# kawshik8/GAN-Image-Captioning

Hardware: AMD Instinct MI355X
Metric: captions/sec (G+D train step) (higher is better)
Workload: dtype bf16; 1 GPU; cfg2: adversarial G+D step, batch 64/GPU, 224x224 images, caption len 20, V=10000, E=H=512, 1-layer LSTM G, CNN-seq D (R=64,F=900), ResNet-50-shaped encoder, --conditional-gan 1; global_batch=64, caption_len=20, image_size=224, vocab=10000, conditional_gan=1, encoder=resnet50, step_impl=fused, parallelism=dp1

## Files before the change

### gan-image-captioning_amd/_lib.py

```python
from __future__ import annotations

import ctypes as C
import os

import torch

from . import build as _build

MAX_LAYERS = 4
MAX_CONVS = 8
F32, BF16 = 0, 1
LOSS_TYPES = {"standard": 0, "JS": 1, "KL": 2, "hinge": 3, "tv": 4, "rsgan": 5}

c_float_p = C.POINTER(C.c_float)
c_void_p = C.c_void_p


class DecoderDims(C.Structure):
    _fields_ = [(n, C.c_int32) for n in ("B", "L", "V", "E", "H", "NL", "dtype")]


class DecoderParams(C.Structure):
    _fields_ = [("embed", c_void_p), ("w_ih", c_void_p * MAX_LAYERS), ("w_hh", c_void_p * MAX_LAYERS),
                ("b_ih", c_void_p * MAX_LAYERS), ("b_hh", c_void_p * MAX_LAYERS), ("w_out", c_void_p), ("b_out", c_void_p)]
# ... 88 lines not shown
                ("o2l_w", c_void_p), ("o2l_b", c_void_p)]


class DiscGrads(C.Structure):
    _fields_ = DiscParams._fields_


class DiscShadow(C.Structure):
    _fields_ = [("emb", c_void_p), ("hw_w", c_void_p), ("f2o_w", c_void_p), ("hw_w_t", c_void_p)]


class DiscState(C.Structure):
    _fields_ = [("emb", c_void_p), ("pooled", c_void_p), ("argmax", c_void_p), ("hpre", c_void_p),
                ("keep", c_void_p), ("ydrop", c_void_p), ("feat", c_void_p)]


class DiscBwdWs(C.Structure):
    _fields_ = [("dfeat", c_void_p), ("dh", c_void_p), ("dydrop", c_void_p), ("dpooled", c_void_p), ("demb", c_void_p)]


class BnRunningDesc(C.Structure):
    _fields_ = [("stats", c_void_p), ("running_mean", c_void_p), ("running_var", c_void_p), ("count", C.c_float),
                ("momentum", C.c_float), ("C", C.c_int32), ("nrep", C.c_int32)]


_P = C.POINTER
_SIGNATURES = {
    "gic_abi_version": (C.c_int, []),
    "gic_last_error": (C.c_char_p, []),
    "gic_debug_route_only": (None, [C.c_int]),
    "gic_debug_last_route": (C.c_char_p, []),
    "gic_gemm": (C.c_int, [c_void_p, c_void_p, c_void_p, C.c_int, C.c_int, C.c_int, C.c_int64, C.c_int64, C.c_int64,
                           C.c_int, C.c_int, C.c_int, C.c_int, c_void_p, C.c_int, C.c_float, c_void_p]),
    "gic_cast2d": (C.c_int, [c_void_p, C.c_int, C.c_int64, c_void_p, C.c_int, C.c_int64, C.c_int64, C.c_int64, c_void_p]),
    "gic_decoder_state_bytes": (C.c_int, [_P(DecoderDims), c_void_p]),
    "gic_decoder_bwd_ws_bytes": (C.c_int, [_P(DecoderDims), c_void_p]),
    "gic_disc_state_bytes": (C.c_int, [_P(DiscDims), c_void_p]),
    "gic_disc_bwd_ws_bytes": (C.c_int, [_P(DiscDims), c_void_p]),
    "gic_decoder_prepare": (C.c_int, [_P(DecoderDims), _P(DecoderParams), _P(DecoderShadow), c_void_p]),
    "gic_decoder_sample_fwd": (C.c_int, [_P(DecoderDims), _P(DecoderParams), _P(DecoderShadow), _P(DecoderState), c_void_p,
                                         c_void_p, C.c_uint64, C.c_float, C.c_int, c_void_p, c_void_p, _P(DecoderSampleOpts), c_void_p]),
    "gic_decoder_forward_tf": (C.c_int, [_P(DecoderDims), _P(DecoderParams), _P(DecoderShadow), _P(DecoderState), c_void_p, c_void_p,
                                         c_void_p, C.c_int, c_void_p, C.c_uint64, C.c_float, C.c_int, c_void_p, c_void_p, c_void_p,
                                         c_void_p, c_void_p, c_void_p]),
    "gic_decoder_forward_tf_bwd": (C.c_int, [_P(DecoderDims), _P(DecoderParams), _P(DecoderShadow), _P(DecoderState), _P(DecoderBwdWs),
                                             c_void_p, c_void_p, c_void_p, C.c_int, c_void_p, C.c_float, C.c_int, _P(DecoderGrads), c_void_p]),
    "gic_decoder_sample_bwd": (C.c_int, [_P(DecoderDims), _P(DecoderParams), _P(DecoderShadow), _P(DecoderState),
                                         _P(DecoderBwdWs), c_void_p, c_void_p, c_void_p, C.c_float, C.c_int,
                                         _P(DecoderGrads), C.c_int, c_void_p, c_void_p]),
    "gic_step_scalars_set": (C.c_int, [c_void_p, _P(StepScalars), c_void_p]),
    "gic_debug_decoder_step": (None, [C.c_int]),
    "gic_decoder_fused_rollout_rows": (C.c_int, [_P(DecoderDims), c_void_p]),
    "gic_decoder_beam_ws_bytes": (C.c_int, [_P(DecoderDims), C.c_int32, c_void_p]),
    "gic_decoder_beam_search": (C.c_int, [_P(DecoderDims), _P(DecoderParams), _P(DecoderShadow), _P(DecoderBeamOpts), c_void_p, c_void_p,
                                          c_void_p, c_void_p, c_void_p, c_void_p]),
    "gic_attn_prepare": (C.c_int, [_P(AttnDims), _P(AttnParams), _P(AttnShadow), c_void_p]),
    "gic_attn_sample_fwd": (C.c_int, [_P(AttnDims), _P(AttnParams), _P(AttnShadow), _P(AttnState), c_void_p, c_void_p, c_void_p, C.c_uint64,
                                      C.c_float, C.c_int, c_void_p, c_void_p, c_void_p, c_void_p, c_void_p, C.c_int, c_void_p]),
    "gic_attn_sample_bwd": (C.c_int, [_P(AttnDims), _P(AttnParams), _P(AttnShadow), _P(AttnState), _P(AttnBwdWs), c_void_p, c_void_p, c_void_p,
                                      c_void_p, C.c_float, C.c_int, _P(AttnGrads), c_void_p, c_void_p]),
    "gic_attn_beam_ws_bytes": (C.c_int, [_P(AttnDims), C.c_int32, c_void_p]),
    "gic_attn_beam_search": (C.c_int, [_P(AttnDims), _P(AttnParams), _P(AttnShadow), _P(DecoderBeamOpts), c_void_p, c_void_p, c_void_p,
                                       c_void_p, c_void_p, c_void_p, c_void_p, c_void_p]),
    "gic_decoder_diverse_beam_search": (C.c_int, [_P(DecoderDims), _P(DecoderParams), _P(DecoderShadow), _P(DiverseBeamOpts), c_void_p,
                                                  c_void_p, c_void_p, c_void_p, c_void_p, c_void_p]),
    "gic_attn_diverse_beam_search": (C.c_int, [_P(AttnDims), _P(AttnParams), _P(AttnShadow), _P(DiverseBeamOpts), c_void_p, c_void_p,
# ... 125 lines not shown
```

### gan-image-captioning_amd/csrc/decoder.hip

```cpp
#include <stdlib.h>

#include "../../include/gicap.h"
#include "decoder_step.h"
#include "kernels.h"

namespace gic {
namespace {

__device__ __forceinline__ float sigmoidf_(float x) { return 1.f / (1.f + expf(-x)); }

template <typename TA>
__global__ void lstm_pointwise_fwd_kernel(const float* __restrict__ gpre, const float* __restrict__ c_prev,
                                          float* __restrict__ gates, float* __restrict__ c_new,
                                          TA* __restrict__ h_next, long ld_next,
                                          TA* __restrict__ h_up, long ld_up,
                                          TA* __restrict__ h_out, long ld_out,
                                          int B, int H) {
  const int idx = blockIdx.x * blockDim.x + threadIdx.x;
  if (idx >= B * H) return;
  const int b = idx / H, j = idx % H;
  const float* g = gpre + (long)b * 4 * H;
  const float i_ = sigmoidf_(g[j]);
  const float f_ = sigmoidf_(g[H + j]);
  const float g_ = tanhf(g[2 * H + j]);
  const float o_ = sigmoidf_(g[3 * H + j]);
  const float c = f_ * c_prev[idx] + i_ * g_;
  const float h = o_ * tanhf(c);
  if (gates) {
    float* go = gates + (long)b * 4 * H;
    go[j] = i_; go[H + j] = f_; go[2 * H + j] = g_; go[3 * H + j] = o_;
  }
  c_new[idx] = c;
  h_next[(long)b * ld_next + j] = from_f32<TA>(h);
  if (h_up) h_up[(long)b * ld_up + j] = from_f32<TA>(h);
  if (h_out) h_out[(long)b * ld_out + j] = from_f32<TA>(h);
}

// ... 536 lines not shown
  } else {
  for (int l = 0; l < NL; ++l) {
    GIC_PROPAGATE(fill_zero(ws->dxh[l], (size_t)(L + 1) * B * c.ldx(l) * sizeof(float), stream));
  }
  for (int t = L - 1; t >= 0; --t) {
    for (int l = NL - 1; l >= 0; --l) {
      const long ld = c.ldx(l);
      const float* dh_a;
      long ld_a;
      if (l == NL - 1) { dh_a = ws->dhout + (long)t * H; ld_a = (long)L * H; }
      else { dh_a = ws->dxh[l + 1] + (long)t * B * c.ldx(l + 1); ld_a = c.ldx(l + 1); }
      const float* dh_b = ws->dxh[l] + (long)(t + 1) * B * ld + c.din(l);
      TA* dg = (TA*)ws->dgates[l] + (long)t * B * 4 * H;
      hipLaunchKernelGGL((lstm_pointwise_bwd_kernel<TA>), dim3(pw_grid), dim3(256), 0, stream, dh_a, ld_a, dh_b, ld,
                         (const float*)(st->gates[l] + (long)t * B * 4 * H), (const float*)(st->c[l] + (long)t * B * H),
                         (const float*)(st->c[l] + (long)(t + 1) * B * H), ws->dc[l], dg, B, H);
      GIC_CHECK_LAUNCH("lstm_pointwise_bwd");
      GemmDesc g;
      g.A = dg; g.lda = 4 * H; g.a_kc = 1;
      if (S->wcat_t[l]) { g.B = S->wcat_t[l]; g.ldb = 4 * H; g.b_kc = 1; }
      else { g.B = S->wcat[l]; g.ldb = ld; g.b_kc = 0; }
      g.C = ws->dxh[l] + (long)t * B * ld; g.ldc = ld; g.c_zeroed = 1;
      g.M = B; g.N = (int)ld; g.K = 4 * H; g.in_dtype = c.dt; g.out_dtype = DT_F32;
      GIC_PROPAGATE(gemm(g, stream));
    }
  }
  }
  for (int l = 0; l < NL; ++l) {
    const long ld = c.ldx(l);
    GemmDesc w;
    w.A = ws->dgates[l]; w.lda = 4 * H; w.a_kc = 0; w.b_kc = 0; w.ldb = ld;
    w.M = 4 * H; w.K = (int)BL; w.in_dtype = c.dt; w.out_dtype = DT_F32;
    w.B = st->xh[l]; w.N = c.din(l); w.C = G->w_ih[l]; w.ldc = c.din(l);
    GIC_PROPAGATE(gemm(w, stream));
    w.B = (const TA*)st->xh[l] + c.din(l); w.N = H; w.C = G->w_hh[l]; w.ldc = H;
    GIC_PROPAGATE(gemm(w, stream));
    GIC_PROPAGATE(colsum(ws->dgates[l], c.dt, 4 * H, BL, 4 * H, G->b_ih[l], G->b_hh[l], 0, stream));
  }
  GIC_PROPAGATE(cast2d(ws->dxh[0], DT_F32, c.ldx(0), G->features, DT_F32, E, B, E, stream));
  return GIC_OK;
}

__global__ void embed_scatter_time_kernel(const float* __restrict__ dxh0, long ld, const int64_t* __restrict__ ids, long ids_stride,
                                          float* __restrict__ dw, int B, int L, int E, int V) {
  const long total = (long)(L - 1) * B * E;
  for (long i = (long)blockIdx.x * blockDim.x + threadIdx.x; i < total; i += (long)gridDim.x * blockDim.x) {
    const int e = (int)(i % E);
    const long r = i / E;
    const int b = (int)(r % B);
    const int t = (int)(r / B) + 1;
    long id = ids[(long)b * ids_stride + (t - 1)];
    id = id < 0 ? 0 : (id >= V ? V - 1 : id);
    atomicAdd(&dw[id * E + e], dxh0[((long)t * B + b) * ld + e]);
  }
}

}

int decoder_output_bwd(int dt, int B, int L, int V, int H, const void* probs, const void* d_out, float temperature, const float* t_dev, int pretrain,
                       void* dlogits_ws, const void* wout, const void* hout, float* dhout, float* d_wout, float* d_bout, hipStream_t stream) {
  const long BL = (long)B * L;
  const void* dlog = pretrain ? d_out : (const void*)dlogits_ws;
  if (!pretrain) {
    const bool al = ((((uintptr_t)probs) | ((uintptr_t)d_out) | ((uintptr_t)dlogits_ws)) & 15) == 0;
    if (dt == DT_F32) {
      if (al && V % 4 == 0 && V <= 256 * 8 * 4)
        hipLaunchKernelGGL((softmax_bwd_vec_kernel<float, 8>), dim3((unsigned)BL), dim3(256), 0, stream, (const float*)probs, (const float*)d_out,
                           (float*)dlogits_ws, temperature, t_dev, V);
      else
        hipLaunchKernelGGL((softmax_bwd_kernel<float>), dim3((unsigned)BL), dim3(256), 0, stream, (const float*)probs, (const float*)d_out,
                           (float*)dlogits_ws, temperature, t_dev, V);
    } else {
      if (al && V % 8 == 0 && V <= 256 * 5 * 8)
        hipLaunchKernelGGL((softmax_bwd_vec_kernel<bf16_t, 5>), dim3((unsigned)BL), dim3(256), 0, stream, (const bf16_t*)probs, (const bf16_t*)d_out,
                           (bf16_t*)dlogits_ws, temperature, t_dev, V);
      else if (al && V % 8 == 0 && V <= 256 * 8 * 8)
        hipLaunchKernelGGL((softmax_bwd_vec_kernel<bf16_t, 8>), dim3((unsigned)BL), dim3(256), 0, stream, (const bf16_t*)probs, (const bf16_t*)d_out,
                           (bf16_t*)dlogits_ws, temperature, t_dev, V);
      else
        hipLaunchKernelGGL((softmax_bwd_kernel<bf16_t>), dim3((unsigned)BL), dim3(256), 0, stream, (const bf16_t*)probs, (const bf16_t*)d_out,
                           (bf16_t*)dlogits_ws, temperature, t_dev, V);
    }
    GIC_CHECK_LAUNCH("softmax_bwd");
  }
  GemmDesc g;
  g.A = dlog; g.lda = V; g.a_kc = 1; g.B = wout; g.ldb = H; g.b_kc = 0; g.C = dhout; g.ldc = H;
  g.M = (int)BL; g.N = H; g.K = V; g.in_dtype = dt; g.out_dtype = DT_F32;
  GIC_PROPAGATE(gemm(g, stream));
  GemmDesc w;
  w.A = dlog; w.lda = V; w.a_kc = 0; w.B = hout; w.ldb = H; w.b_kc = 0; w.C = d_wout; w.ldc = H;
  w.M = V; w.N = H; w.K = (int)BL; w.in_dtype = dt; w.out_dtype = DT_F32;
  GIC_PROPAGATE(gemm(w, stream));
  return colsum(dlog, dt, V, BL, V, d_bout, nullptr, 0, stream);
}

int lstm_pointwise_fwd(int dt, const float* gpre, const float* c_prev, float* c_new, void* h_next, long ld_next, void* h_up, long ld_up,
                       int rows, int H, hipStream_t stream) {
  const dim3 grid((unsigned)cdiv((long)rows * H, 256));
  if (dt == DT_F32)
    hipLaunchKernelGGL((lstm_pointwise_fwd_kernel<float>), grid, dim3(256), 0, stream, gpre, c_prev, (float*)nullptr, c_new, (float*)h_next, ld_next,
                       (float*)h_up, ld_up, (float*)nullptr, 0l, rows, H);
  else
    hipLaunchKernelGGL((lstm_pointwise_fwd_kernel<bf16_t>), grid, dim3(256), 0, stream, gpre, c_prev, (float*)nullptr, c_new, (bf16_t*)h_next,
                       ld_next, (bf16_t*)h_up, ld_up, (bf16_t*)nullptr, 0l, rows, H);
  GIC_CHECK_LAUNCH("lstm_pointwise_fwd");
  return GIC_OK;
}

int embed_scatter_time(const float* dx, long ld, const int64_t* ids, float* d_embed, int B, int L, int E, int V, hipStream_t stream, long ids_stride) {
  if (ids_stride <= 0) ids_stride = L;
  GIC_PROPAGATE(fill_zero(d_embed, (size_t)V * E * sizeof(float), stream));
  if (L > 1 && det_mode())
    return det_scatter(dx, DT_F32, ld, B, ids, B, ids_stride, 1, (long)(L - 1) * B, d_embed, E, 1, E, V, stream);
  if (L > 1) {
    const long total = (long)(L - 1) * B * E;
    const int grid = (int)((total + 255) / 256 > 2048 ? 2048 : (total + 255) / 256);
    hipLaunchKernelGGL(embed_scatter_time_kernel, dim3(grid), dim3(256), 0, stream, dx, ld, ids, ids_stride, d_embed, B, L, E, V);
    GIC_CHECK_LAUNCH("embed_scatter_time");
  }
  return GIC_OK;
}

}

using namespace gic;
// ... 316 lines not shown
```

### gan-image-captioning_amd/csrc/disc.hip

```cpp
#include <stdlib.h>
#include "../../include/gicap.h"
#include "kernels.h"

namespace gic {
namespace {

constexpr int kMaxTaps = 32;
constexpr int kOutDim = 100;
constexpr int kOutPad = 104;

struct ConvMeta {
  int nconv, F, Fp, s;
  int fsize[GIC_MAX_CONVS], nfilt[GIC_MAX_CONVS], foff[GIC_MAX_CONVS];
  const float* w[GIC_MAX_CONVS];
  const float* b[GIC_MAX_CONVS];
  float* dw[GIC_MAX_CONVS];
  float* db[GIC_MAX_CONVS];
};

__device__ __forceinline__ int conv_of(const ConvMeta& cm, int col) {
  int k = 0;
  while (k + 1 < cm.nconv && col >= cm.foff[k + 1]) ++k;
  return k;
}

__global__ void disc_emb_gather_kernel(const float* __restrict__ w, const int64_t* __restrict__ ids, float* __restrict__ emb,
                                       long rows, int De, int V) {
  const long total = rows * De;
  for (long i = (long)blockIdx.x * blockDim.x + threadIdx.x; i < total; i += (long)gridDim.x * blockDim.x) {
    const long r = i / De;
    const int e = (int)(i % De);
    long id = ids[r];
    id = id < 0 ? 0 : (id >= V ? V - 1 : id);
    emb[i] = w[(long)e * V + id];
  }
// ... 698 lines not shown
               const float* d_logits, const gic_disc_grads* G, int accumulate, void* d_inp, long ld_dinp, hipStream_t stream) {
  const long MR = c.rowsBR;
  if (G && !accumulate) {
    GIC_PROPAGATE(fill_zero(G->o2l_w, kOutDim * sizeof(float), stream));
    GIC_PROPAGATE(fill_zero(G->o2l_b, sizeof(float), stream));
    for (int k = 0; k < c.cm.nconv; ++k) {
      GIC_PROPAGATE(fill_zero(G->conv_w[k], (size_t)c.cm.nfilt[k] * c.cm.fsize[k] * c.s * sizeof(float), stream));
      GIC_PROPAGATE(fill_zero(G->conv_b[k], (size_t)c.cm.nfilt[k] * sizeof(float), stream));
    }
    if (inp_ids) GIC_PROPAGATE(fill_zero(G->emb, (size_t)c.De * c.V * sizeof(float), stream));
  }
  const bool det = G && det_mode();
  const long dy_floats = MR * c.Fp;
  int out_blocks = 256;
  if (det && (long)out_blocks * (kOutDim + 1) > dy_floats) out_blocks = (int)(dy_floats / (kOutDim + 1));
  if (out_blocks < 1) out_blocks = 1;
  const bool out_part = det && out_blocks > 1;
  hipLaunchKernelGGL((disc_out_bwd_kernel<TA>), dim3(out_blocks), dim3(256), 0, stream, d_logits, (const float*)st->feat, P->o2l_w,
                     (TA*)ws->dfeat, G ? G->o2l_w : nullptr, G ? G->o2l_b : nullptr, MR, out_part ? ws->dydrop : nullptr);
  GIC_CHECK_LAUNCH("disc_out_bwd");
  if (out_part) {
    hipLaunchKernelGGL(disc_out_fold_kernel, dim3(1), dim3(128), 0, stream, (const float*)ws->dydrop, out_blocks, G->o2l_w, G->o2l_b);
    GIC_CHECK_LAUNCH("disc_out_fold");
  }
  {
    GemmDesc g;
    g.A = ws->dfeat; g.lda = kOutPad; g.a_kc = 1; g.B = S->f2o_w; g.ldb = c.Fp; g.b_kc = 0; g.C = ws->dydrop; g.ldc = c.Fp;
    g.M = (int)MR; g.N = c.Fp; g.K = kOutPad; g.in_dtype = c.dt; g.out_dtype = DT_F32;
    GIC_PROPAGATE(gemm(g, stream));
    if (G) {
      GemmDesc w;
      w.A = ws->dfeat; w.lda = kOutPad; w.a_kc = 0; w.B = st->ydrop; w.ldb = c.Fp; w.b_kc = 0; w.C = G->f2o_w; w.ldc = c.F;
      w.M = kOutDim; w.N = c.F; w.K = (int)MR; w.in_dtype = c.dt; w.out_dtype = DT_F32; w.accumulate = accumulate;
      GIC_PROPAGATE(gemm(w, stream));
      GIC_PROPAGATE(colsum(ws->dfeat, c.dt, kOutPad, MR, kOutDim, G->f2o_b, nullptr, accumulate, stream, (float*)ws->dh,
                           (long)(MR * c.Fp * dtype_size(c.dt) / sizeof(float))));
    }
  }
  const bool hb_vec = MR * c.Fp / 8 < (1l << 31) && ((((uintptr_t)ws->dydrop) | ((uintptr_t)st->hpre) | ((uintptr_t)st->pooled) | ((uintptr_t)ws->dh) |
                                                     ((uintptr_t)ws->dpooled)) & 15) == 0 && (!train || (((uintptr_t)st->keep) & 7) == 0);
  if (hb_vec)
    hipLaunchKernelGGL((disc_highway_bwd_vec_kernel<TA>), dim3(grid1d(MR * c.Fp / 8)), dim3(256), 0, stream, (const float*)ws->dydrop,
                       train ? (const uint8_t*)st->keep : nullptr, c.keep_scale(train), (const float*)st->hpre,
                       (const TA*)st->pooled, (TA*)ws->dh, ws->dpooled, (unsigned)(MR * c.Fp / 8), c.F, c.Fp / 8);
  else
    hipLaunchKernelGGL((disc_highway_bwd_kernel<TA>), dim3(grid1d(MR * c.Fp)), dim3(256), 0, stream, (const float*)ws->dydrop,
                       train ? (const uint8_t*)st->keep : nullptr, c.keep_scale(train), (const float*)st->hpre,
                       (const TA*)st->pooled, (TA*)ws->dh, ws->dpooled, MR, c.F, c.Fp);
  GIC_CHECK_LAUNCH("disc_highway_bwd");
  {
    GemmDesc g;
    g.A = ws->dh; g.lda = c.Fp; g.a_kc = 1; g.B = S->hw_w_t ? S->hw_w_t : S->hw_w; g.ldb = c.Fp; g.b_kc = S->hw_w_t ? 1 : 0;
    g.C = ws->dpooled; g.ldc = c.Fp;
    g.M = (int)MR; g.N = c.Fp; g.K = c.Fp; g.in_dtype = c.dt; g.out_dtype = DT_F32; g.accumulate = 1;
    GIC_PROPAGATE(gemm(g, stream));
    if (G) {
      GemmDesc w;
      w.A = ws->dh; w.lda = c.Fp; w.a_kc = 0; w.B = st->pooled; w.ldb = c.Fp; w.b_kc = 0; w.C = G->hw_w; w.ldc = c.F;
      w.M = c.F; w.N = c.F; w.K = (int)MR; w.in_dtype = c.dt; w.out_dtype = DT_F32; w.accumulate = accumulate;
      GIC_PROPAGATE(gemm(w, stream));
      GIC_PROPAGATE(colsum(ws->dh, c.dt, c.Fp, MR, c.F, G->hw_b, nullptr, accumulate, stream, ws->dydrop, (long)(MR * c.Fp)));
    }
  }
  if (G) {
    int gy = cdiv(MR, 4 * 8);
    gy = gy > 64 ? 64 : gy;
    int mt = 0;
    for (int k = 0; k < c.cm.nconv; ++k) mt = c.cm.fsize[k] * c.s > mt ? c.cm.fsize[k] * c.s : mt;
    static const bool no_lds = getenv("GIC_NO_DISC_BWDW_LDS") != nullptr;
    const bool lds = mt <= 8 && c.s == 1 && c.R <= 64 && c.R <= c.De && MR % c.R == 0 && c.L <= 64 && !no_lds;
    const int ncap = (int)(MR / c.R);
    const int mt1 = (mt <= 8 ? 8 : kMaxTaps) + 1;
    int rows_y = lds ? (ncap < 64 ? ncap : 64) : gy;
    if (det && (long)rows_y * c.F * mt1 > dy_floats) rows_y = (int)(dy_floats / ((long)c.F * mt1));
    if (rows_y < 1) rows_y = 1;
    gy = lds ? gy : rows_y;
    float* part = det && rows_y > 1 ? ws->dydrop : nullptr;
    if (lds) {
      hipLaunchKernelGGL((disc_conv_pool_bwd_w_lds_kernel<TA, 8>), dim3(cdiv(c.F, 64), rows_y), dim3(256),
                         (size_t)c.R * ((c.L + 8) | 1) * sizeof(float), stream, (const float*)ws->dpooled, (const TA*)st->pooled,
                         (const uint8_t*)st->argmax, (const float*)st->emb, c.cm, c.L, c.De, c.R, ncap, part);
    } else if (mt <= 8)
      hipLaunchKernelGGL((disc_conv_pool_bwd_w_kernel<TA, 8>), dim3(cdiv(c.F, 64), gy), dim3(256), 0, stream, (const float*)ws->dpooled,
                         (const TA*)st->pooled, (const uint8_t*)st->argmax, (const float*)st->emb, c.cm, c.L, c.De, c.R, MR, part);
    else
      hipLaunchKernelGGL((disc_conv_pool_bwd_w_kernel<TA, kMaxTaps>), dim3(cdiv(c.F, 64), gy), dim3(256), 0, stream, (const float*)ws->dpooled,
                         (const TA*)st->pooled, (const uint8_t*)st->argmax, (const float*)st->emb, c.cm, c.L, c.De, c.R, MR, part);
    GIC_CHECK_LAUNCH("disc_conv_pool_bwd_w");
    if (part) {
      hipLaunchKernelGGL(disc_wgrad_fold_kernel, dim3(cdiv((long)c.F * mt1, 256)), dim3(256), 0, stream, (const float*)ws->dydrop, rows_y, mt1, c.cm);
      GIC_CHECK_LAUNCH("disc_wgrad_fold");
    }
  }
  const int n_out = c.L * c.s;
  size_t conv_w_total = 0;
  for (int k = 0; k < c.cm.nconv; ++k) conv_w_total += (size_t)c.cm.nfilt[k] * c.cm.fsize[k] * c.s;
  const size_t bwd_x_lds = ((size_t)3 * c.Fp + (size_t)(n_out >= 256 ? 1 : 256 / n_out) * n_out + conv_w_total) * sizeof(float);
  GIC_CHECK_ARG(bwd_x_lds <= 160 * 1024, "disc_bwd: conv weights (%zu floats) do not fit the LDS staging", conv_w_total);
  int max_taps_x = 0;
  for (int k = 0; k < c.cm.nconv; ++k) max_taps_x = c.cm.fsize[k] * c.s > max_taps_x ? c.cm.fsize[k] * c.s : max_taps_x;
  if (n_out <= 32 && c.F <= 1024 && max_taps_x <= 8) {
    static const int rpb_env = [] { const char* e = getenv("GIC_BWDX_RPB"); return e ? atoi(e) : 0; }();
    const int rpb = rpb_env > 0 ? rpb_env : (MR >= 2048 ? 4 : 1);
    hipLaunchKernelGGL((disc_conv_pool_bwd_x_small_kernel<TA, 32, 8>), dim3((unsigned)cdiv(MR, rpb)), dim3(256), (size_t)n_out * 256 * sizeof(float), stream,
                       (const float*)ws->dpooled, (const TA*)st->pooled, (const uint8_t*)st->argmax, c.cm, c.L, c.De, c.R,
                       (TA*)ws->demb, (int)MR, rpb);
  } else {
    hipLaunchKernelGGL((disc_conv_pool_bwd_x_kernel<TA>), dim3((unsigned)MR), dim3(256), bwd_x_lds, stream,
                       (const float*)ws->dpooled, (const TA*)st->pooled, (const uint8_t*)st->argmax, c.cm, c.L, c.De, c.R, (TA*)ws->demb);
  }
  GIC_CHECK_LAUNCH("disc_conv_pool_bwd_x");
  if (G) {
    if (inp_ids && inp_soft) {
      const long half = c.rowsBL / 2;
      if (det_mode()) {
        GIC_PROPAGATE(det_scatter(ws->demb, c.dt, c.De, 0, inp_ids, (int)half, 1, 0, half, G->emb, 1, c.V, c.De, c.V, stream));
      } else {
        hipLaunchKernelGGL(disc_emb_scatter_kernel, dim3(grid1d(half * c.De)), dim3(256), 0, stream, (const float*)nullptr,
                           (const void*)ws->demb, c.dt, inp_ids, G->emb, half, c.De, c.V);
        GIC_CHECK_LAUNCH("disc_emb_scatter");
      }
      GemmDesc w;
      w.A = (const char*)ws->demb + (size_t)half * c.De * dtype_size(c.dt); w.lda = c.De; w.a_kc = 0; w.B = inp_soft; w.ldb = ld_inp; w.b_kc = 0;
      w.C = G->emb; w.ldc = c.V;
      w.M = c.De; w.N = c.V; w.K = (int)half; w.in_dtype = c.dt; w.out_dtype = DT_F32; w.accumulate = 1;
      GIC_PROPAGATE(gemm(w, stream));
    } else if (inp_ids) {
      if (det_mode()) {
        GIC_PROPAGATE(det_scatter(ws->demb, c.dt, c.De, 0, inp_ids, (int)c.rowsBL, 1, 0, c.rowsBL, G->emb, 1, c.V, c.De, c.V, stream));
      } else {
        hipLaunchKernelGGL(disc_emb_scatter_kernel, dim3(grid1d(c.rowsBL * c.De)), dim3(256), 0, stream, (const float*)nullptr,
                           (const void*)ws->demb, c.dt, inp_ids, G->emb, c.rowsBL, c.De, c.V);
        GIC_CHECK_LAUNCH("disc_emb_scatter");
      }
    } else {
      GemmDesc w;
      w.A = ws->demb; w.lda = c.De; w.a_kc = 0; w.B = inp_soft; w.ldb = ld_inp; w.b_kc = 0; w.C = G->emb; w.ldc = c.V;
      w.M = c.De; w.N = c.V; w.K = (int)c.rowsBL; w.in_dtype = c.dt; w.out_dtype = DT_F32; w.accumulate = accumulate;
      GIC_PROPAGATE(gemm(w, stream));
    }
  }
  if (d_inp) {
    GemmDesc g;
    g.A = ws->demb; g.lda = c.De; g.a_kc = 1; g.B = S->emb; g.ldb = c.V; g.b_kc = 0; g.C = d_inp; g.ldc = ld_dinp;
    g.M = (int)c.rowsBL; g.N = c.V; g.K = c.De; g.in_dtype = c.dt; g.out_dtype = c.dt;
    GIC_PROPAGATE(gemm(g, stream));
  }
  return GIC_OK;
}

}
}

using namespace gic;

extern "C" {

int gic_disc_state_bytes(const gic_disc_dims* dims, uint64_t* out) {
  DCtx c;
  GIC_PROPAGATE(make_ctx(dims, nullptr, nullptr, c));
  GIC_CHECK_ARG(out, "disc_state_bytes: null out");
  const uint64_t a = dtype_size(c.dt), MR = c.rowsBR, Fp = c.Fp;
  out[0] = (uint64_t)c.rowsBL * c.De * 4;
  out[1] = MR * Fp * a;
  out[2] = MR * Fp;
  out[3] = MR * Fp * 4;
  out[4] = MR * Fp;
  out[5] = MR * Fp * a;
  out[6] = MR * kOutDim * 4;
  return GIC_OK;
}

// ... 82 lines not shown
```

### gan-image-captioning_amd/csrc/util.hip

```cpp
#include <stdarg.h>
#include <stdio.h>

#include "../../include/gicap.h"
#include "kernels.h"

namespace gic {

static thread_local char g_last_error[512] = "";

void set_last_error(const char* fmt, ...) {
  va_list ap;
  va_start(ap, fmt);
  vsnprintf(g_last_error, sizeof(g_last_error), fmt, ap);
  va_end(ap);
}

static thread_local bool g_route_only = false;
static thread_local char g_route[kRouteLen] = "";
bool route_only() { return g_route_only; }
char* route_line() { return g_route; }

namespace {

template <typename TA>
__global__ void transpose2d_kernel(const TA* __restrict__ in, TA* __restrict__ out, int rows, int cols) {
  __shared__ TA tile[32][33];
  const int c0 = blockIdx.x * 32, r0 = blockIdx.y * 32;
  const int tx = threadIdx.x & 31, ty = threadIdx.x >> 5;
  for (int j = ty; j < 32; j += 8)
    if (r0 + j < rows && c0 + tx < cols) tile[j][tx] = in[(long)(r0 + j) * cols + c0 + tx];
  __syncthreads();
  for (int j = ty; j < 32; j += 8)
    if (c0 + j < cols && r0 + tx < rows) out[(long)(c0 + j) * rows + r0 + tx] = tile[tx][j];
}

template <typename TS, typename TD>
__global__ void cast2d_kernel(const TS* __restrict__ src, long lds, TD* __restrict__ dst, long ldd, long rows, long cols) {
// ... 246 lines not shown
  return GIC_OK;
}

int embedding_bwd(const float* d_out, const int64_t* ids, float* d_weight, long n, int V, int E, int zero_first,
                  hipStream_t stream) {
  GIC_CHECK_ARG(d_out && ids && d_weight, "embedding_bwd: null pointer");
  if (zero_first) GIC_PROPAGATE(fill_zero(d_weight, (size_t)V * E * sizeof(float), stream));
  if (n * E == 0) return GIC_OK;
  if (det_mode()) return det_scatter(d_out, DT_F32, E, 0, ids, (int)n, 1, 0, n, d_weight, E, 1, E, V, stream);
  hipLaunchKernelGGL(embedding_bwd_kernel, dim3(grid_for(n * E)), dim3(256), 0, stream, d_out, ids, d_weight, n, V, E);
  GIC_CHECK_LAUNCH("embedding_bwd");
  return GIC_OK;
}

}

extern "C" {

int gic_abi_version(void) { return GIC_ABI_VERSION; }
const char* gic_last_error(void) { return gic::g_last_error; }
void gic_debug_route_only(int on) { gic::g_route_only = on != 0; }
const char* gic_debug_last_route(void) { return gic::g_route; }

int gic_gemm(const void* A, const void* B, void* C, int M, int N, int K, int64_t lda, int64_t ldb, int64_t ldc,
             int a_kc, int b_kc, int in_dtype, int out_dtype, const float* bias, int accumulate, float alpha,
             void* stream) {
  gic::GemmDesc d;
  d.A = A; d.B = B; d.C = C; d.M = M; d.N = N; d.K = K; d.lda = lda; d.ldb = ldb; d.ldc = ldc;
  d.a_kc = a_kc; d.b_kc = b_kc; d.in_dtype = in_dtype; d.out_dtype = out_dtype;
  d.bias = bias; d.accumulate = accumulate; d.alpha = alpha;
  return gic::gemm(d, (hipStream_t)stream);
}

int gic_cast2d(const void* src, int src_dtype, int64_t lds, void* dst, int dst_dtype, int64_t ldd, int64_t rows,
               int64_t cols, void* stream) {
  return gic::cast2d(src, src_dtype, lds, dst, dst_dtype, ldd, rows, cols, (hipStream_t)stream);
}

int gic_embedding_fwd(const float* weight, const int64_t* ids, float* out, int64_t n, int32_t V, int32_t E, void* stream) {
  return gic::embedding_fwd(weight, ids, out, n, V, E, (hipStream_t)stream);
}

int gic_embedding_bwd(const float* d_out, const int64_t* ids, float* d_weight, int64_t n, int32_t V, int32_t E,
                      int zero_first, void* stream) {
  return gic::embedding_bwd(d_out, ids, d_weight, n, V, E, zero_first, (hipStream_t)stream);
}

}
```

### gan-image-captioning_amd/engine.py

```python
from __future__ import annotations

import ctypes as C
import os
from typing import Dict, List, Optional, Sequence, Tuple

import torch

from . import _lib as L

TORCH_DTYPE = {L.F32: torch.float32, L.BF16: torch.bfloat16}
DTYPE_BY_NAME = {"fp32": L.F32, "f32": L.F32, "float32": L.F32, "bf16": L.BF16, "bfloat16": L.BF16}

_param_epoch = 0


def set_deterministic(on: bool) -> None:
    L.check(L.load().gic_set_deterministic(int(bool(on))), "gic_set_deterministic")


def deterministic() -> bool:
    return bool(L.load().gic_get_deterministic())


def bump_param_epoch() -> None:
# ... 74 lines not shown

def _arr(ctype, n, values):
    a = (ctype * n)()
    for i, v in enumerate(values):
        a[i] = v
    return a


def _key(params: Sequence[torch.Tensor]):
    return tuple((p.data_ptr(), p._version) for p in params) + (_param_epoch,)


class StepScalarsBuffer:

    def __init__(self, device):
        self.buf = torch.zeros(C.sizeof(L.StepScalars), dtype=torch.uint8, device=device)
        self.ptr = self.buf.data_ptr()

    def set(self, temperature: float, seeds) -> None:
        v = L.StepScalars()
        v.temperature = float(temperature)
        for i, sd in enumerate(seeds):
            v.seed[i] = int(sd) & (2 ** 64 - 1)
        L.check(L.load().gic_step_scalars_set(self.ptr, C.byref(v), stream_ptr()), "gic_step_scalars_set")


def gemm(A, B, Cout, M, N, K, lda, ldb, ldc, a_kc=True, b_kc=True, bias=None, accumulate=False, alpha=1.0):
    require_gpu(A, B, Cout)
    in_dt = L.F32 if A.dtype == torch.float32 else L.BF16
    out_dt = L.F32 if Cout.dtype == torch.float32 else L.BF16
    L.check(L.load().gic_gemm(ptr(A), ptr(B), ptr(Cout), M, N, K, lda, ldb, ldc, int(a_kc), int(b_kc), in_dt, out_dt,
                              ptr(bias), int(accumulate), float(alpha), stream_ptr()), "gic_gemm")
    return Cout


def cast2d(src: torch.Tensor, dst: torch.Tensor, rows: int, cols: int, lds: int, ldd: int):
    require_gpu(src, dst)
    sd = L.F32 if src.dtype == torch.float32 else L.BF16
    dd = L.F32 if dst.dtype == torch.float32 else L.BF16
    L.check(L.load().gic_cast2d(ptr(src), sd, lds, ptr(dst), dd, ldd, rows, cols, stream_ptr()), "gic_cast2d")
    return dst


def _to_act(t: torch.Tensor, act: torch.dtype) -> torch.Tensor:
    t = t.contiguous()
    if t.dtype == act:
        return t
    n = t.shape[-1]
    return cast2d(t, torch.empty(t.shape, device=t.device, dtype=act), t.numel() // n, n, n, n)


def embedding_fwd(weight: torch.Tensor, ids: torch.Tensor) -> torch.Tensor:
    require_gpu(weight, ids)
    ids = ids.contiguous()
    out = torch.empty(ids.numel(), weight.shape[1], device=weight.device, dtype=torch.float32)
    L.check(L.load().gic_embedding_fwd(ptr(weight), ptr(ids), ptr(out), ids.numel(), weight.shape[0], weight.shape[1],
                                       stream_ptr()), "gic_embedding_fwd")
    return out.view(*ids.shape, weight.shape[1])


def embedding_bwd(d_out: torch.Tensor, ids: torch.Tensor, V: int, d_weight: Optional[torch.Tensor] = None,
                  zero_first: bool = True) -> torch.Tensor:
    require_gpu(d_out, ids)
    E = d_out.shape[-1]
    d_out = d_out.contiguous()
    ids = ids.contiguous()
# ... 1057 lines not shown
```

### include/gicap.h

```cpp
#ifndef GICAP_H_
#define GICAP_H_

#include <stdint.h>

#ifdef __cplusplus
extern "C" {
#endif

#define GIC_ABI_VERSION 5
#define GIC_MAX_LAYERS 4
#define GIC_MAX_CONVS 8

enum gic_status {
  GIC_STATUS_OK = 0,
  GIC_STATUS_INVALID_ARG = -1,
  GIC_STATUS_UNSUPPORTED = -2,
  GIC_STATUS_LAUNCH = -3,
  GIC_STATUS_WORKSPACE = -4
};
enum gic_dtype { GIC_F32 = 0, GIC_BF16 = 1 };
enum gic_loss_type {
  GIC_LOSS_STANDARD = 0, GIC_LOSS_JS = 1, GIC_LOSS_KL = 2, GIC_LOSS_HINGE = 3, GIC_LOSS_TV = 4, GIC_LOSS_RSGAN = 5
};

int gic_abi_version(void);
const char* gic_last_error(void);

void gic_debug_route_only(int on);
const char* gic_debug_last_route(void);

#define GIC_STEP_SEEDS 6
typedef struct gic_step_scalars {
  float temperature;
  uint32_t reserved;
  uint64_t seed[GIC_STEP_SEEDS];
} gic_step_scalars;
int gic_step_scalars_set(gic_step_scalars* dev, const gic_step_scalars* host_values, void* stream);

int gic_gemm(const void* A, const void* B, void* C, int M, int N, int K, int64_t lda, int64_t ldb, int64_t ldc,
             int a_kc, int b_kc, int in_dtype, int out_dtype, const float* bias, int accumulate, float alpha,
             void* stream);

int gic_cast2d(const void* src, int src_dtype, int64_t lds, void* dst, int dst_dtype, int64_t ldd,
               int64_t rows, int64_t cols, void* stream);

typedef struct gic_decoder_dims {
  int32_t B, L, V, E, H, NL;
  int32_t dtype;
} gic_decoder_dims;

typedef struct gic_decoder_params {
  const float* embed;
  const float* w_ih[GIC_MAX_LAYERS];
  const float* w_hh[GIC_MAX_LAYERS];
  const float* b_ih[GIC_MAX_LAYERS];
  const float* b_hh[GIC_MAX_LAYERS];
  const float* w_out;
  const float* b_out;
} gic_decoder_params;

typedef struct gic_decoder_grads {
  float* embed;
  float* w_ih[GIC_MAX_LAYERS];
  float* w_hh[GIC_MAX_LAYERS];
  float* b_ih[GIC_MAX_LAYERS];
  float* b_hh[GIC_MAX_LAYERS];
  float* w_out;
  float* b_out;
  float* features;
} gic_decoder_grads;

typedef struct gic_decoder_shadow {
  void* wcat[GIC_MAX_LAYERS];
  float* bsum[GIC_MAX_LAYERS];
// ... 376 lines not shown
```

Measured before the change: 26260 captions/s.

## Add dedicated MFMA weight-gradient GEMM kernel with split-K and route wgrad calls

Adds a specialized bf16 weight-gradient GEMM kernel for the K-major x K-major case. It uses 128x128 tiles, buffer-load-to-LDS DMA with 4-stage pipelining, transposing LDS reads (ds_read_b64_tr_b16), MFMA 16x16x32, and a cost-model-chosen split-K with atomic accumulation. Decoder LSTM, output projection and discriminator weight-gradient GEMMs now try this path first and fall back to the generic gemm. The intent is to cut the cost of the long-K, small-MN wgrad reductions. In exchange it brings atomic nondeterminism, an extra zeroing kernel when split, and hand-written asm that is easy to get subtly wrong.

New measurement: 26490 captions/s (median of 6 runs). Within noise of the previous version (+0.9%).

```diff
diff --git a/gan-image-captioning_amd/_lib.py b/gan-image-captioning_amd/_lib.py
--- a/gan-image-captioning_amd/_lib.py
+++ b/gan-image-captioning_amd/_lib.py
@@ -144,6 +144,7 @@
     "gic_debug_last_route": (C.c_char_p, []),
     "gic_gemm": (C.c_int, [c_void_p, c_void_p, c_void_p, C.c_int, C.c_int, C.c_int, C.c_int64, C.c_int64, C.c_int64,
                            C.c_int, C.c_int, C.c_int, C.c_int, c_void_p, C.c_int, C.c_float, c_void_p]),
+    "gic_wgrad": (C.c_int, [c_void_p, c_void_p, c_void_p, C.c_int, C.c_int, C.c_int, C.c_int64, C.c_int64, C.c_int64, C.c_int, C.c_int, c_void_p]),
     "gic_cast2d": (C.c_int, [c_void_p, C.c_int, C.c_int64, c_void_p, C.c_int, C.c_int64, C.c_int64, C.c_int64, c_void_p]),
     "gic_decoder_state_bytes": (C.c_int, [_P(DecoderDims), c_void_p]),
     "gic_decoder_bwd_ws_bytes": (C.c_int, [_P(DecoderDims), c_void_p]),
diff --git a/gan-image-captioning_amd/csrc/decoder.hip b/gan-image-captioning_amd/csrc/decoder.hip
--- a/gan-image-captioning_amd/csrc/decoder.hip
+++ b/gan-image-captioning_amd/csrc/decoder.hip
@@ -3,6 +3,7 @@
 #include "../../include/gicap.h"
 #include "decoder_step.h"
 #include "kernels.h"
+#include "wgrad.h"
 
 namespace gic {
 namespace {
@@ -605,9 +606,9 @@
     w.A = ws->dgates[l]; w.lda = 4 * H; w.a_kc = 0; w.b_kc = 0; w.ldb = ld;
     w.M = 4 * H; w.K = (int)BL; w.in_dtype = c.dt; w.out_dtype = DT_F32;
     w.B = st->xh[l]; w.N = c.din(l); w.C = G->w_ih[l]; w.ldc = c.din(l);
-    GIC_PROPAGATE(gemm(w, stream));
+    GIC_PROPAGATE(wgrad_or_gemm(w, stream));
     w.B = (const TA*)st->xh[l] + c.din(l); w.N = H; w.C = G->w_hh[l]; w.ldc = H;
-    GIC_PROPAGATE(gemm(w, stream));
+    GIC_PROPAGATE(wgrad_or_gemm(w, stream));
     GIC_PROPAGATE(colsum(ws->dgates[l], c.dt, 4 * H, BL, 4 * H, G->b_ih[l], G->b_hh[l], 0, stream));
   }
   GIC_PROPAGATE(cast2d(ws->dxh[0], DT_F32, c.ldx(0), G->features, DT_F32, E, B, E, stream));
@@ -663,7 +664,7 @@
   GemmDesc w;
   w.A = dlog; w.lda = V; w.a_kc = 0; w.B = hout; w.ldb = H; w.b_kc = 0; w.C = d_wout; w.ldc = H;
   w.M = V; w.N = H; w.K = (int)BL; w.in_dtype = dt; w.out_dtype = DT_F32;
-  GIC_PROPAGATE(gemm(w, stream));
+  GIC_PROPAGATE(wgrad_or_gemm(w, stream));
   return colsum(dlog, dt, V, BL, V, d_bout, nullptr, 0, stream);
 }
 
diff --git a/gan-image-captioning_amd/csrc/disc.hip b/gan-image-captioning_amd/csrc/disc.hip
--- a/gan-image-captioning_amd/csrc/disc.hip
+++ b/gan-image-captioning_amd/csrc/disc.hip
@@ -1,6 +1,7 @@
 #include <stdlib.h>
 #include "../../include/gicap.h"
 #include "kernels.h"
+#include "wgrad.h"
 
 namespace gic {
 namespace {
@@ -765,7 +766,7 @@
       GemmDesc w;
       w.A = ws->dfeat; w.lda = kOutPad; w.a_kc = 0; w.B = st->ydrop; w.ldb = c.Fp; w.b_kc = 0; w.C = G->f2o_w; w.ldc = c.F;
       w.M = kOutDim; w.N = c.F; w.K = (int)MR; w.in_dtype = c.dt; w.out_dtype = DT_F32; w.accumulate = accumulate;
-      GIC_PROPAGATE(gemm(w, stream));
+      GIC_PROPAGATE(wgrad_or_gemm(w, stream));
       GIC_PROPAGATE(colsum(ws->dfeat, c.dt, kOutPad, MR, kOutDim, G->f2o_b, nullptr, accumulate, stream, (float*)ws->dh,
                            (long)(MR * c.Fp * dtype_size(c.dt) / sizeof(float))));
     }
@@ -791,7 +792,7 @@
       GemmDesc w;
       w.A = ws->dh; w.lda = c.Fp; w.a_kc = 0; w.B = st->pooled; w.ldb = c.Fp; w.b_kc = 0; w.C = G->hw_w; w.ldc = c.F;
       w.M = c.F; w.N = c.F; w.K = (int)MR; w.in_dtype = c.dt; w.out_dtype = DT_F32; w.accumulate = accumulate;
-      GIC_PROPAGATE(gemm(w, stream));
+      GIC_PROPAGATE(wgrad_or_gemm(w, stream));
       GIC_PROPAGATE(colsum(ws->dh, c.dt, c.Fp, MR, c.F, G->hw_b, nullptr, accumulate, stream, ws->dydrop, (long)(MR * c.Fp)));
     }
   }
@@ -857,7 +858,7 @@
       w.A = (const char*)ws->demb + (size_t)half * c.De * dtype_size(c.dt); w.lda = c.De; w.a_kc = 0; w.B = inp_soft; w.ldb = ld_inp; w.b_kc = 0;
       w.C = G->emb; w.ldc = c.V;
       w.M = c.De; w.N = c.V; w.K = (int)half; w.in_dtype = c.dt; w.out_dtype = DT_F32; w.accumulate = 1;
-      GIC_PROPAGATE(gemm(w, stream));
+      GIC_PROPAGATE(wgrad_or_gemm(w, stream));
     } else if (inp_ids) {
       if (det_mode()) {
         GIC_PROPAGATE(det_scatter(ws->demb, c.dt, c.De, 0, inp_ids, (int)c.rowsBL, 1, 0, c.rowsBL, G->emb, 1, c.V, c.De, c.V, stream));
@@ -870,7 +871,7 @@
       GemmDesc w;
       w.A = ws->demb; w.lda = c.De; w.a_kc = 0; w.B = inp_soft; w.ldb = ld_inp; w.b_kc = 0; w.C = G->emb; w.ldc = c.V;
       w.M = c.De; w.N = c.V; w.K = (int)c.rowsBL; w.in_dtype = c.dt; w.out_dtype = DT_F32; w.accumulate = accumulate;
-      GIC_PROPAGATE(gemm(w, stream));
+      GIC_PROPAGATE(wgrad_or_gemm(w, stream));
     }
   }
   if (d_inp) {
diff --git a/gan-image-captioning_amd/csrc/util.hip b/gan-image-captioning_amd/csrc/util.hip
--- a/gan-image-captioning_amd/csrc/util.hip
+++ b/gan-image-captioning_amd/csrc/util.hip
@@ -3,6 +3,7 @@
 
 #include "../../include/gicap.h"
 #include "kernels.h"
+#include "wgrad.h"
 
 namespace gic {
 
@@ -315,6 +316,14 @@
   return gic::gemm(d, (hipStream_t)stream);
 }
 
+int gic_wgrad(const void* A, const void* B, float* C, int M, int N, int K, int64_t lda, int64_t ldb, int64_t ldc, int in_dtype, int accumulate,
+              void* stream) {
+  gic::WgradDesc d;
+  d.A = A; d.B = B; d.C = C; d.M = M; d.N = N; d.K = K; d.lda = lda; d.ldb = ldb; d.ldc = ldc;
+  d.in_dtype = in_dtype; d.accumulate = accumulate;
+  return gic::wgrad(d, (hipStream_t)stream);
+}
+
 int gic_cast2d(const void* src, int src_dtype, int64_t lds, void* dst, int dst_dtype, int64_t ldd, int64_t rows,
                int64_t cols, void* stream) {
   return gic::cast2d(src, src_dtype, lds, dst, dst_dtype, ldd, rows, cols, (hipStream_t)stream);
diff --git a/gan-image-captioning_amd/csrc/wgrad.h b/gan-image-captioning_amd/csrc/wgrad.h
--- /dev/null
+++ b/gan-image-captioning_amd/csrc/wgrad.h
@@ -0,0 +1,26 @@
+#pragma once
+#include "common.h"
+#include "gemm.h"
+
+namespace gic {
+
+struct WgradDesc {
+  const void* A = nullptr;
+  const void* B = nullptr;
+  float* C = nullptr;
+  int M = 0, N = 0, K = 0;
+  long lda = 0, ldb = 0, ldc = 0;
+  int in_dtype = DT_BF16;
+  int accumulate = 0;
+  int c_zeroed = 0;
+};
+
+struct WgradPlan { int bm, bn, tiles, splits, per, zero_grid; };
+
+bool select_wgrad(const WgradDesc& d, WgradPlan& p);
+
+int wgrad(const WgradDesc& d, hipStream_t stream);
+
+int wgrad_or_gemm(const GemmDesc& d, hipStream_t stream);
+
+}
diff --git a/gan-image-captioning_amd/csrc/wgrad.hip b/gan-image-captioning_amd/csrc/wgrad.hip
--- /dev/null
+++ b/gan-image-captioning_amd/csrc/wgrad.hip
@@ -0,0 +1,257 @@
+#include "wgrad.h"
+#include "kernels.h"
+
+#include <stdio.h>
+#include <stdlib.h>
+#include <type_traits>
+
+namespace gic {
+
+namespace {
+
+struct WgradArgs {
+  const void* A; const void* B; float* C;
+  int M, N, K, lda, ldb;
+  long ldc;
+  int per, accumulate;
+};
+
+constexpr int kBK = 32;
+
+template <int BM, int BN>
+__global__ __launch_bounds__(512) void wgrad_kernel(const WgradArgs a) {
+  static_assert(BM == 128 && BN == 128, "one 16-byte chunk per thread and operand: 32 rows x 16 chunks = 512 threads; 2 + 4 fragments per wave");
+  constexpr int BK = kBK, NS = 4, NL = 2;
+  constexpr int TM = BM / 64, TN = BN / 32;
+  constexpr int RA = BM * 2, RB = BN * 2;
+  constexpr int A_BYTES = BK * RA, B_BYTES = BK * RB, STAGE = A_BYTES + B_BYTES;
+  constexpr unsigned OOB = 0x80000000u;
+  static_assert(RA == RB && (NS - 1) * STAGE + 4 * RA < 65536, "one immediate per fragment read");
+  __shared__ __attribute__((aligned(16))) unsigned char smem[NS * STAGE];
+
+  const int tid = threadIdx.x, lane = tid & 63, w = tid >> 6;
+  const int wr = w >> 1, wc = w & 1;
+  const int lr = lane & 15, lg = lane >> 4;
+  const int M = a.M, N = a.N, K = a.K;
+
+  const int tiles_m = (M + BM - 1) / BM;
+  const int bid = xcd_run(blockIdx.x, gridDim.x);
+  const int bm0 = (bid % tiles_m) * BM;
+  const int bn0 = (bid / tiles_m) * BN;
+
+  const int nk = (K + BK - 1) / BK;
+  const int kt0 = blockIdx.y * a.per;
+  const int kt1 = min(nk, kt0 + a.per);
+  const int k_end = min(K, kt1 * BK);
+  const unsigned a_bytes = ((unsigned)(k_end - 1) * (unsigned)a.lda + (unsigned)((M + 7) & ~7)) * 2u;
+  const unsigned b_bytes = ((unsigned)(k_end - 1) * (unsigned)a.ldb + (unsigned)((N + 7) & ~7)) * 2u;
+  const __amdgpu_buffer_rsrc_t rsA = __builtin_amdgcn_make_buffer_rsrc((void*)a.A, 0, (int)a_bytes, 0x00020000);
+  const __amdgpu_buffer_rsrc_t rsB = __builtin_amdgcn_make_buffer_rsrc((void*)a.B, 0, (int)b_bytes, 0x00020000);
+
+  const int drow = tid >> 4;
+  const int dchunk = (tid & 15) ^ (((drow & 3) << 1) | (((drow >> 3) & 1) << 3));
+  const int am = bm0 + dchunk * 8, bn = bn0 + dchunk * 8;
+  unsigned va = am < M ? ((unsigned)(kt0 * BK + drow) * (unsigned)a.lda + (unsigned)am) * 2u : OOB;
+  unsigned vb = bn < N ? ((unsigned)(kt0 * BK + drow) * (unsigned)a.ldb + (unsigned)bn) * 2u : OOB;
+  const unsigned va_step = (unsigned)(BK * 2) * (unsigned)a.lda, vb_step = (unsigned)(BK * 2) * (unsigned)a.ldb;
+  const int wbase = __builtin_amdgcn_readfirstlane(w) * 1024;
+
+  auto issue = [&](auto st_c) {
+    constexpr int ST = decltype(st_c)::value;
+    __builtin_amdgcn_raw_ptr_buffer_load_lds(rsA, (lds_void_ptr)(smem + ST * STAGE + wbase), 16, (int)va, 0, 0, 0);
+    __builtin_amdgcn_raw_ptr_buffer_load_lds(rsB, (lds_void_ptr)(smem + ST * STAGE + A_BYTES + wbase), 16, (int)vb, 0, 0, 0);
+    va += va_step; vb += vb_step;
+  };
+
+  f32x4 acc[TM][TN];
+#pragma unroll
+  for (int i = 0; i < TM; ++i)
+#pragma unroll
+    for (int j = 0; j < TN; ++j) acc[i][j] = (f32x4){0.f, 0.f, 0.f, 0.f};
+
+  const unsigned lds0 = (unsigned)(uintptr_t)(__attribute__((address_space(3))) unsigned char*)smem;
+  const int fq = lr >> 2, fp = lr & 3;
+  const int fsw = (fq << 1) | ((lg & 1) << 3);
+  const int frow = lg * 8 + fq;
+  auto frag_addr = [&](int c0) { return (unsigned)(frow * RA + ((((c0 >> 3) + (fp >> 1)) ^ fsw) << 4) + (fp & 1) * 8); };
+  const unsigned adA0 = lds0 + frag_addr(wr * (BM / 4)), adA1 = lds0 + frag_addr(wr * (BM / 4) + 16);
+  const unsigned adB0 = lds0 + A_BYTES + frag_addr(wc * (BN / 2)), adB1 = lds0 + A_BYTES + frag_addr(wc * (BN / 2) + 16);
+  const unsigned adB2 = lds0 + A_BYTES + frag_addr(wc * (BN / 2) + 32), adB3 = lds0 + A_BYTES + frag_addr(wc * (BN / 2) + 48);
+
+  struct Frags { bf16x4 r[12]; };
+  auto read_frags = [&](auto st_c, Frags& f) {
+    constexpr int ST = decltype(st_c)::value;
+    const unsigned x0 = adA0, x1 = adA1, y0 = adB0, y1 = adB1, y2 = adB2, y3 = adB3;
+    asm volatile(
+        "ds_read_b64_tr_b16 %0, %12 offset:%18\n\t"
+        "ds_read_b64_tr_b16 %1, %12 offset:%19\n\t"
+        "ds_read_b64_tr_b16 %2, %13 offset:%18\n\t"
+        "ds_read_b64_tr_b16 %3, %13 offset:%19\n\t"
+        "ds_read_b64_tr_b16 %4, %14 offset:%18\n\t"
+        "ds_read_b64_tr_b16 %5, %14 offset:%19\n\t"
+        "ds_read_b64_tr_b16 %6, %15 offset:%18\n\t"
+        "ds_read_b64_tr_b16 %7, %15 offset:%19\n\t"
+        "ds_read_b64_tr_b16 %8, %16 offset:%18\n\t"
+        "ds_read_b64_tr_b16 %9, %16 offset:%19\n\t"
+        "ds_read_b64_tr_b16 %10, %17 offset:%18\n\t"
+        "ds_read_b64_tr_b16 %11, %17 offset:%19"
+        : "=&v"(f.r[0]), "=&v"(f.r[1]), "=&v"(f.r[2]), "=&v"(f.r[3]), "=&v"(f.r[4]), "=&v"(f.r[5]), "=&v"(f.r[6]), "=&v"(f.r[7]), "=&v"(f.r[8]),
+          "=&v"(f.r[9]), "=&v"(f.r[10]), "=&v"(f.r[11])
+        : "v"(x0), "v"(x1), "v"(y0), "v"(y1), "v"(y2), "v"(y3), "n"(ST * STAGE), "n"(ST * STAGE + 4 * RA)
+        : "memory");
+  };
+  auto frags_arrived = [&](Frags& f) {
+    asm volatile("s_waitcnt lgkmcnt(0)"
+                 : "+v"(f.r[0]), "+v"(f.r[1]), "+v"(f.r[2]), "+v"(f.r[3]), "+v"(f.r[4]), "+v"(f.r[5]), "+v"(f.r[6]), "+v"(f.r[7]), "+v"(f.r[8]),
+                   "+v"(f.r[9]), "+v"(f.r[10]), "+v"(f.r[11])
+                 :
+                 : "memory");
+  };
+  auto mfma = [&](const Frags& f) {
+    bf16x8 fa[TM], fb[TN];
+#pragma unroll
+    for (int t = 0; t < TM; ++t) fa[t] = __builtin_shufflevector(f.r[2 * t], f.r[2 * t + 1], 0, 1, 2, 3, 4, 5, 6, 7);
+#pragma unroll
+    for (int t = 0; t < TN; ++t) fb[t] = __builtin_shufflevector(f.r[2 * TM + 2 * t], f.r[2 * TM + 2 * t + 1], 0, 1, 2, 3, 4, 5, 6, 7);
+#pragma unroll
+    for (int i = 0; i < TM; ++i)
+#pragma unroll
+      for (int j = 0; j < TN; ++j)
+        acc[i][j] = __builtin_amdgcn_mfma_f32_16x16x32_bf16(fa[i], fb[j], acc[i][j], 0, 0, 0);
+  };
+
+  std::integral_constant<int, 0> s0; std::integral_constant<int, 1> s1; std::integral_constant<int, 2> s2; std::integral_constant<int, 3> s3;
+  const bool dma_first = __builtin_amdgcn_readfirstlane(w) < 4;
+  auto step = [&](auto next_c, auto fill_c, const Frags& cur, Frags& nxt) {
+    asm volatile("s_waitcnt vmcnt(%0)" ::"n"((NS - 2) * NL) : "memory");
+    __builtin_amdgcn_s_barrier();
+    if (dma_first) issue(fill_c);
+    read_frags(next_c, nxt);
+    __builtin_amdgcn_sched_barrier(0);
+    mfma(cur);
+    __builtin_amdgcn_sched_barrier(0);
+    if (!dma_first) issue(fill_c);
+    frags_arrived(nxt);
+  };
+  issue(s0); issue(s1); issue(s2);
+  asm volatile("s_waitcnt vmcnt(%0)" ::"n"((NS - 2) * NL) : "memory");
+  __builtin_amdgcn_s_barrier();
+  issue(s3);
+  Frags f0, f1;
+  read_frags(s0, f0);
+  frags_arrived(f0);
+  for (int trips = (kt1 - kt0 + NS - 1) / NS; trips > 0; --trips) {
+    step(s1, s0, f0, f1);
+    step(s2, s1, f1, f0);
+    step(s3, s2, f0, f1);
+    step(s0, s3, f1, f0);
+  }
+  asm volatile("s_waitcnt vmcnt(0)" ::: "memory");
+
+  float* __restrict__ C = a.C;
+  const bool split = gridDim.y > 1;
+  auto each = [&](auto&& f) {
+#pragma unroll
+    for (int i = 0; i < TM; ++i)
+#pragma unroll
+      for (int j = 0; j < TN; ++j) {
+        const int n = bn0 + wc * (BN / 2) + j * 16 + lr;
+        const int mb = bm0 + wr * (BM / 4) + i * 16 + lg * 4;
+#pragma unroll
+        for (int r = 0; r < 4; ++r)
+          if (n < N && mb + r < M) f(C + (long)(mb + r) * a.ldc + n, acc[i][j][r]);
+      }
+  };
+  if (split) each([](float* p, float v) { atomicAdd(p, v); });
+  else if (a.accumulate) each([](float* p, float v) { *p += v; });
+  else each([](float* p, float v) { *p = v; });
+}
+
+__global__ void wgrad_zero_kernel(float* __restrict__ C, long ldc, int M, int N) {
+  const long total = (long)M * N;
+  for (long i = (long)blockIdx.x * blockDim.x + threadIdx.x; i < total; i += (long)gridDim.x * blockDim.x)
+    C[(i / N) * ldc + (i % N)] = 0.f;
+}
+
+bool aligned16(const void* p) { return (((uintptr_t)p) & 15) == 0; }
+
+void write_route(const WgradPlan& p) {
+  snprintf(route_line(), kRouteLen, "wgrad<%d,%d> grid=%dx%d block=512 lds=0 splits=%d per=%d zero=%d", p.bm, p.bn, p.tiles, p.splits, p.splits,
+           p.per, p.zero_grid);
+}
+
+void launch_wgrad(const WgradDesc& d, const WgradPlan& p, hipStream_t stream) {
+  if (p.zero_grid) hipLaunchKernelGGL(wgrad_zero_kernel, dim3(p.zero_grid), dim3(256), 0, stream, d.C, d.ldc, d.M, d.N);
+  WgradArgs a;
+  a.A = d.A; a.B = d.B; a.C = d.C; a.M = d.M; a.N = d.N; a.K = d.K; a.lda = (int)d.lda; a.ldb = (int)d.ldb; a.ldc = d.ldc;
+  a.per = p.per; a.accumulate = d.accumulate;
+  hipLaunchKernelGGL((wgrad_kernel<128, 128>), dim3(p.tiles, p.splits), dim3(512), 0, stream, a);
+}
+
+}
+
+bool select_wgrad(const WgradDesc& d, WgradPlan& p) {
+  static const bool off = [] { const char* e = getenv("GIC_NO_WGRAD"); return e && atoi(e) != 0; }();
+  if (off || d.in_dtype != DT_BF16 || det_mode()) return false;
+  if (d.M < 1 || d.N < 1 || d.K < 256) return false;
+  if (!aligned16(d.A) || !aligned16(d.B) || (((uintptr_t)d.C) & 3) || d.lda % 8 || d.ldb % 8 || d.lda < d.M || d.ldb < d.N || d.ldc < d.N) return false;
+  const long a_elems = (long)(d.K - 1) * d.lda + ((d.M + 7) & ~7), b_elems = (long)(d.K - 1) * d.ldb + ((d.N + 7) & ~7);
+  if (a_elems * 2 >= (1l << 31) || b_elems * 2 >= (1l << 31)) return false;
+  p.bm = p.bn = 128;
+  p.tiles = cdiv(d.M, p.bm) * cdiv(d.N, p.bn);
+  const int nk = cdiv(d.K, kBK);
+  constexpr double kTileUs = 0.25, kWgMBus = 0.024, kHbmMBus = 5.0, kAtomicMBus = 0.8, kZeroMBus = 3.0;
+  const double c_mb = (double)d.M * d.N * 4e-6, ab_mb = ((double)d.M + d.N) * d.K * 2e-6;
+  int splits = 1;
+  double best = 0.;
+  for (int s = 1; s <= 16 && s <= (nk / 8 > 1 ? nk / 8 : 1); ++s) {
+    const int per = cdiv(nk, s), wgs = p.tiles * cdiv(nk, per);
+    const double loop = per * kTileUs * (wgs > 256 ? wgs / 256. : 1.), rate = wgs * kWgMBus < kHbmMBus ? wgs * kWgMBus : kHbmMBus;
+    double t = loop > ab_mb / rate ? loop : ab_mb / rate;
+    if (s > 1) t += s * c_mb / kAtomicMBus + ((d.accumulate || d.c_zeroed) ? 0. : c_mb / kZeroMBus);
+    if (s == 1 || t < best) { best = t; splits = s; }
+  }
+  { const char* e = getenv("GIC_WGRAD_SPLITS"); if (e && atoi(e) > 0) splits = atoi(e) < nk ? atoi(e) : nk; }
+  p.per = cdiv(nk, splits);
+  p.splits = cdiv(nk, p.per);
+  p.zero_grid = 0;
+  if (p.splits > 1 && !d.accumulate && !d.c_zeroed) {
+    const long blocks = ((long)d.M * d.N + 255) / 256;
+    p.zero_grid = (int)(blocks > 1024 ? 1024 : blocks);
+  }
+  return true;
+}
+
+int wgrad(const WgradDesc& d, hipStream_t stream) {
+  static const bool log = getenv("GIC_GEMM_LOG") != nullptr;
+  const bool probe = route_only();
+  if (probe) route_line()[0] = 0;
+  GIC_CHECK_ARG(d.A && d.B && d.C, "wgrad: null operand");
+  GIC_CHECK_ARG(d.M >= 0 && d.N >= 0 && d.K >= 0, "wgrad: negative dim");
+  WgradPlan p;
+  if (!select_wgrad(d, p)) {
+    if (probe) snprintf(route_line(), kRouteLen, "unsupported");
+    return GIC_ERR_UNSUPPORTED;
+  }
+  if (log || probe) {
+    write_route(p);
+    if (log) fprintf(stderr, "[wgrad] M=%d N=%d K=%d acc=%d -> %s\n", d.M, d.N, d.K, d.accumulate, route_line());
+  }
+  if (probe) return GIC_OK;
+  launch_wgrad(d, p, stream);
+  GIC_CHECK_LAUNCH("wgrad");
+  return GIC_OK;
+}
+
+int wgrad_or_gemm(const GemmDesc& g, hipStream_t stream) {
+  if (!g.a_kc && !g.b_kc && !g.conv && g.epi == EPI_PLAIN && g.out_dtype == DT_F32 && !g.bias && g.alpha == 1.f && !g.no_split && g.A && g.B && g.C) {
+    WgradDesc d;
+    d.A = g.A; d.B = g.B; d.C = (float*)g.C; d.M = g.M; d.N = g.N; d.K = g.K; d.lda = g.lda; d.ldb = g.ldb; d.ldc = g.ldc;
+    d.in_dtype = g.in_dtype; d.accumulate = g.accumulate; d.c_zeroed = g.c_zeroed;
+    const int rc = wgrad(d, stream);
+    if (rc != GIC_ERR_UNSUPPORTED) return rc;
+  }
+  return gemm(g, stream);
+}
+
+}
diff --git a/gan-image-captioning_amd/engine.py b/gan-image-captioning_amd/engine.py
--- a/gan-image-captioning_amd/engine.py
+++ b/gan-image-captioning_amd/engine.py
@@ -130,6 +130,16 @@
     L.check(L.load().gic_gemm(ptr(A), ptr(B), ptr(Cout), M, N, K, lda, ldb, ldc, int(a_kc), int(b_kc), in_dt, out_dt,
                               ptr(bias), int(accumulate), float(alpha), stream_ptr()), "gic_gemm")
     return Cout
+
+
+def wgrad(A, B, Cout, M, N, K, lda, ldb, ldc, accumulate=False) -> bool:
+    require_gpu(A, B, Cout)
+    in_dt = L.F32 if A.dtype == torch.float32 else L.BF16
+    rc = L.load().gic_wgrad(ptr(A), ptr(B), ptr(Cout), M, N, K, lda, ldb, ldc, in_dt, int(accumulate), stream_ptr())
+    if rc == L.ERR_UNSUPPORTED:
+        return False
+    L.check(rc, "gic_wgrad")
+    return True
 
 
 def cast2d(src: torch.Tensor, dst: torch.Tensor, rows: int, cols: int, lds: int, ldd: int):
diff --git a/include/gicap.h b/include/gicap.h
--- a/include/gicap.h
+++ b/include/gicap.h
@@ -40,6 +40,9 @@
 int gic_gemm(const void* A, const void* B, void* C, int M, int N, int K, int64_t lda, int64_t ldb, int64_t ldc,
              int a_kc, int b_kc, int in_dtype, int out_dtype, const float* bias, int accumulate, float alpha,
              void* stream);
+
+int gic_wgrad(const void* A, const void* B, float* C, int M, int N, int K, int64_t lda, int64_t ldb, int64_t ldc,
+              int in_dtype, int accumulate, void* stream);
 
 int gic_cast2d(const void* src, int src_dtype, int64_t lds, void* dst, int dst_dtype, int64_t ldd,
                int64_t rows, int64_t cols, void* stream);
```
